# sangminwoo/Temporal-Span-Proposal-Network-VidVRD

Measured on AMD Instinct MI355X. Metric: tracklet-pairs/sec scored (N=32, T=150, D=2048), higher is better.
Workload: dtype f32

## Files before the change

temporal-span-proposal-network-vidvrd_amd/csrc/tspn_device.h:

```cpp
#pragma once
#include <hip/hip_runtime.h>

namespace tspn_dev {

typedef float f32x2 __attribute__((ext_vector_type(2)));
typedef float f32x4 __attribute__((ext_vector_type(4)));
typedef float f32x16 __attribute__((ext_vector_type(16)));
typedef __bf16 bf16x2 __attribute__((ext_vector_type(2)));
typedef __bf16 bf16x4 __attribute__((ext_vector_type(4)));
typedef __bf16 bf16x8 __attribute__((ext_vector_type(8)));
typedef _Float16 f16x8 __attribute__((ext_vector_type(8)));
typedef short s16x2 __attribute__((ext_vector_type(2)));
typedef unsigned u32x4 __attribute__((ext_vector_type(4)));

template <int AUX = 0>
__device__ __forceinline__ void glds16(const void* g, void* l) {
  __builtin_amdgcn_global_load_lds((const __attribute__((address_space(1))) void*)g,
                                   (__attribute__((address_space(3))) void*)l, 16, 0, AUX);
}
__device__ __forceinline__ void glds4(const void* g, void* l) {
  __builtin_amdgcn_global_load_lds((const __attribute__((address_space(1))) void*)g,
                                   (__attribute__((address_space(3))) void*)l, 4, 0, 0);
}

constexpr int kBufferFlags = 0x00020000;
constexpr int kBufferUnbounded = 0x7fffffff;
__device__ __forceinline__ __amdgpu_buffer_rsrc_t buffer_rsrc(const void* p, int bytes) {
  return __builtin_amdgcn_make_buffer_rsrc(const_cast<void*>(p), 0, bytes, kBufferFlags);
}
__device__ __forceinline__ __amdgpu_buffer_rsrc_t buffer_rsrc_unbounded(const void* p) {
  return buffer_rsrc(p, kBufferUnbounded);
}

__device__ __forceinline__ void bglds16(__amdgpu_buffer_rsrc_t rsrc, unsigned voff, int soff, void* l) {
  __builtin_amdgcn_raw_ptr_buffer_load_lds(rsrc, (__attribute__((address_space(3))) void*)l, 16, (int)voff, soff, 0, 0);
}

template <int OFF>
__device__ __forceinline__ void load_wfrag(f32x4& dst, unsigned lane_off, const char* base) {
  asm volatile("global_load_dwordx4 %0, %1, %2 offset:%3" : "=v"(dst) : "v"(lane_off), "s"(base), "n"(OFF) : "memory");
}
template <int VM>
__device__ __forceinline__ void wait_w(f32x4& r) {
  asm volatile("s_waitcnt vmcnt(%1)" : "+v"(r) : "n"(VM));
}
template <int VM>
__device__ __forceinline__ void wait_w(f32x4& r0, f32x4& r1) {
  asm volatile("s_waitcnt vmcnt(%2)" : "+v"(r0), "+v"(r1) : "n"(VM));
}
template <int N>
__device__ __forceinline__ void wait_vmcnt() {
  asm volatile("s_waitcnt vmcnt(%0)" ::"n"(N) : "memory");
}

__device__ __forceinline__ int xcd_remap(int id, int n) {
  const int q8 = n >> 3, r8 = n & 7, xcd = id & 7;
  return (xcd < r8 ? xcd * (q8 + 1) : r8 * (q8 + 1) + (xcd - r8) * q8) + (id >> 3);
}
__device__ __forceinline__ void grouped_tile(int wg, int GM, int tiles_m, int tiles_n, int& tile_m, int& tile_n) {
  const int group_sz = GM * tiles_n;
  const int group = wg / group_sz;
  const int first_m = group * GM;
  const int gm = min(GM, tiles_m - first_m);
  const int in_group = wg - group * group_sz;
  tile_m = first_m + in_group % gm;
  tile_n = in_group / gm;
}

}
```

temporal-span-proposal-network-vidvrd_amd/csrc/tspn_wino63.hip:

```cpp
#include <algorithm>
#include <atomic>
#include <type_traits>

#include "tspn_common.h"
#include "tspn_device.h"

namespace {

using namespace tspn_dev;

constexpr int NW = 4;
constexpr int THREADS = 64 * NW;
constexpr int BM = 128;
constexpr int ST = 32;
constexpr int SWG = 64;
constexpr int KC = 8;
constexpr int NJ = 8;
constexpr int VROW = ST * 4;
constexpr int VCH = 2 * NJ * VROW;
constexpr int VHALF = 4 * VCH;
constexpr int VSS = 2 * VHALF;
constexpr int NVB = 2;
constexpr int NPIECE = 16;
constexpr size_t SMEM_BYTES = sizeof(float) * NVB * VSS;
// ... 177 lines not shown
    if (JP == 1) { load_wfrag<2048>(ap[2], aoff, base); load_wfrag<3072>(ap[3], aoff, base); }
    if (JP == 2) { load_wfrag<0>(ap[4], aoff, base + 4096); load_wfrag<1024>(ap[5], aoff, base + 4096); }
    if (JP == 3) { load_wfrag<2048>(ap[6], aoff, base + 4096); load_wfrag<3072>(ap[7], aoff, base + 4096); }
  };
  using P0 = std::integral_constant<int, 0>;
  using P1 = std::integral_constant<int, 1>;
  using P2 = std::integral_constant<int, 2>;
  using P3 = std::integral_constant<int, 3>;
  auto mfma_pair = [&](const f32x4* ap, int ja, int jb, int S1, int slot) {
#pragma unroll
    for (int e = 0; e < 4; ++e) {
      acc[0][ja] = __builtin_amdgcn_mfma_f32_32x32x2f32(ap[ja][e], v[0][ja][e], acc[0][ja], 0, 0, 0);
      acc[0][jb] = __builtin_amdgcn_mfma_f32_32x32x2f32(ap[jb][e], v[0][jb][e], acc[0][jb], 0, 0, 0);
      acc[1][ja] = __builtin_amdgcn_mfma_f32_32x32x2f32(ap[ja][e], v[1][ja][e], acc[1][ja], 0, 0, 0);
      if (S1 >= 0) {
        __builtin_amdgcn_sched_barrier(0);
        stage_piece(S1, 4 * slot + e);
        __builtin_amdgcn_sched_barrier(0);
      }
      acc[1][jb] = __builtin_amdgcn_mfma_f32_32x32x2f32(ap[jb][e], v[1][jb][e], acc[1][jb], 0, 0, 0);
    }
  };

#pragma unroll
  for (int k = 0; k < NPIECE; ++k) stage_piece(0, k);
  asm volatile("s_waitcnt vmcnt(0)" ::: "memory");
  __syncthreads();
#pragma unroll
  for (int j = 0; j < NJ; ++j) load_v(vlane, 0, j);
  load_a_pair(a[0], P0{}, abase); load_a_pair(a[0], P1{}, abase); load_a_pair(a[0], P2{}, abase); load_a_pair(a[0], P3{}, abase);
  abase += NJ * 1024;
  load_a_pair(a[1], P0{}, abase); load_a_pair(a[1], P1{}, abase); load_a_pair(a[1], P2{}, abase); load_a_pair(a[1], P3{}, abase);
  abase += NJ * 1024;
  __builtin_amdgcn_sched_barrier(0);

  auto chunk_body = [&](auto cl_tag, const float* vcur, const float* vnext, int S, auto has1_tag, auto has2_tag,
                        auto more_tag) {
    constexpr int CL = decltype(cl_tag)::value;
    constexpr bool HAS1 = decltype(has1_tag)::value;
    constexpr bool HAS2 = decltype(has2_tag)::value;
    constexpr bool MORE = decltype(more_tag)::value;
    constexpr int PAR = CL & 1;
    constexpr int N1 = (HAS1 ? 8 : 0) + ((MORE && CL == 1) ? NPIECE : 0);
    constexpr int N2 = (MORE && CL == 2) ? 6 : 2;
    constexpr int N0 = (HAS2 ? 2 : 0) + ((MORE && CL == 0) ? 4 : 0);
    const int S1 = (MORE && CL == 0) ? S + 1 : -1;
    const float* vn = CL == 3 ? vnext : vcur;
    constexpr int NCL = (CL + 1) & 3;
    f32x4* ap = a[PAR];
    wait_w<3 * N2 + N1>(ap[0], ap[1]);
    mfma_pair(ap, 0, 1, S1, 0);
    if (HAS2) load_a_pair(ap, P0{}, abase);
    if (HAS1) { load_v(vn, NCL, 0); load_v(vn, NCL, 1); }
    __builtin_amdgcn_sched_barrier(0);
    wait_w<2 * N2 + N1 + N0>(ap[2], ap[3]);
    mfma_pair(ap, 2, 3, S1, 1);
    if (HAS2) load_a_pair(ap, P1{}, abase);
    if (HAS1) { load_v(vn, NCL, 2); load_v(vn, NCL, 3); }
    __builtin_amdgcn_sched_barrier(0);
    wait_w<N2 + N1 + 2 * N0>(ap[4], ap[5]);
    mfma_pair(ap, 4, 5, S1, 2);
    if (HAS2) load_a_pair(ap, P2{}, abase);
    if (HAS1) { load_v(vn, NCL, 4); load_v(vn, NCL, 5); }
    __builtin_amdgcn_sched_barrier(0);
    wait_w<N1 + 3 * N0>(ap[6], ap[7]);
    mfma_pair(ap, 6, 7, S1, 3);
    if (HAS2) {
      load_a_pair(ap, P3{}, abase);
      abase += NJ * 1024;
    }
    if (HAS1) { load_v(vn, NCL, 6); load_v(vn, NCL, 7); }
    __builtin_amdgcn_sched_barrier(0);
    if (MORE && CL == 2) {
      asm volatile("s_waitcnt lgkmcnt(0)" ::: "memory");
      __builtin_amdgcn_s_barrier();
      __builtin_amdgcn_sched_barrier(0);
    }
  };
  {
    using TT = std::true_type;
    using FF = std::false_type;
    using C0 = std::integral_constant<int, 0>;
    using C1 = std::integral_constant<int, 1>;
    using C2 = std::integral_constant<int, 2>;
    using C3 = std::integral_constant<int, 3>;
    int S = 0;
    for (; S + 1 < nsuper; ++S) {
      const float* vcur = vlane + (S & 1) * VSS;
      const float* vnext = vlane + ((S + 1) & 1) * VSS;
      chunk_body(C0{}, vcur, vnext, S, TT{}, TT{}, TT{});
      chunk_body(C1{}, vcur, vnext, S, TT{}, TT{}, TT{});
      chunk_body(C2{}, vcur, vnext, S, TT{}, TT{}, TT{});
      chunk_body(C3{}, vcur, vnext, S, TT{}, TT{}, TT{});
    }
    const float* vcur = vlane + (S & 1) * VSS;
    chunk_body(C0{}, vcur, vcur, S, TT{}, TT{}, FF{});
    chunk_body(C1{}, vcur, vcur, S, TT{}, TT{}, FF{});
    chunk_body(C2{}, vcur, vcur, S, TT{}, FF{}, FF{});
    chunk_body(C3{}, vcur, vcur, S, FF{}, FF{}, FF{});
  }

#pragma unroll
  for (int cb = 0; cb < 2; ++cb) {
    const int64_t Sx = S0 + ST * cb + li;
    if (Sx < nsext) {
      const int64_t b = Sx / nq;
      const int q = (int)(Sx - b * nq);
      const int t = 6 * q;
      float* ycol = y + (b * M) * (int64_t)ldy + t;
#pragma unroll
      for (int e = 0; e < 16; ++e) {
        const int m = m0 + wave * 32 + (e & 3) + 8 * (e >> 2) + 4 * kh;
        if (m < M) {
          const float p12 = acc[cb][1][e] + acc[cb][2][e], m12 = acc[cb][1][e] - acc[cb][2][e];
          const float p34 = acc[cb][3][e] + acc[cb][4][e], m34 = acc[cb][3][e] - acc[cb][4][e];
          const float p56 = acc[cb][5][e] + acc[cb][6][e], m56 = acc[cb][5][e] - acc[cb][6][e];
          float o[6];
          o[0] = acc[cb][0][e] + p12 + p34 + p56;
          o[1] = m12 + 2.f * m34 + 0.5f * m56;
          o[2] = p12 + 4.f * p34 + 0.25f * p56;
          o[3] = m12 + 8.f * m34 + 0.125f * m56;
          o[4] = p12 + 16.f * p34 + 0.0625f * p56;
          o[5] = m12 + 32.f * m34 + 0.03125f * m56 + acc[cb][7][e];
          if (bias != nullptr) {
            const float bb = bias[m];
#pragma unroll
            for (int i = 0; i < 6; ++i) o[i] += bb;
          }
          if (relu) {
#pragma unroll
            for (int i = 0; i < 6; ++i) o[i] = tspn::relu_f32(o[i]);
          }
          float* dst = ycol + (int64_t)m * ldy;
          if (vec2) {
            *reinterpret_cast<f32x2*>(dst) = f32x2{o[0], o[1]};
            *reinterpret_cast<f32x2*>(dst + 2) = f32x2{o[2], o[3]};
            *reinterpret_cast<f32x2*>(dst + 4) = f32x2{o[4], o[5]};
          } else {
#pragma unroll
            for (int i = 0; i < 6; ++i)
              if (t + i < T) dst[i] = o[i];
          }
        }
      }
    }
  }
}

constexpr int F_BM = 256, F_BN = 256;
constexpr int F_THREADS = 512;
constexpr int F_ST = 4 * 2 * 256 * 16;
constexpr int F_NST = 4;
constexpr size_t F_SMEM = (size_t)F_NST * F_ST;
constexpr size_t F_SMEM_ALL = F_SMEM + 2 * 256 * sizeof(int);
static_assert(TSPN_WINO63_GM > 0 && TSPN_WINO63_GM < 256, "the contraction's GM argument carries the tail split and the piece form above bit 7");
constexpr size_t F_PARK_PER_TILE = (size_t)7 * F_THREADS * 128 * sizeof(float);

__device__ __forceinline__ int split_exponent(double mx) {
  if (!(mx > 0.0) || !(mx <= 1.7976931348623157e308)) return 0;
  int k;
  (void)frexp(mx, &k);
  return 15 - k;
}

__device__ __forceinline__ double wino63_u(int j, double g0, double g1, double g2) {
  switch (j) {
    case 0: return g0;
    case 1: return -2.0 / 9.0 * (g0 + g1 + g2);
    case 2: return -2.0 / 9.0 * (g0 - g1 + g2);
    case 3: return g0 / 90.0 + g1 / 45.0 + 2.0 * g2 / 45.0;
    case 4: return g0 / 90.0 - g1 / 45.0 + 2.0 * g2 / 45.0;
    case 5: return (32.0 * g0 + 16.0 * g1 + 8.0 * g2) / 45.0;
    case 6: return (32.0 * g0 - 16.0 * g1 + 8.0 * g2) / 45.0;
    default: return g2;
  }
}

__global__ void pack_wino63_frag_kernel(const float* __restrict__ W, int64_t M, int64_t Cin, int64_t split,
                                        int16_t* __restrict__ out) {
  const int64_t Mp = split ? 2 * M : M, Cp = split ? split : Cin;
  const int64_t ncg = Cp / 8;
  const int64_t o = blockIdx.x * (int64_t)blockDim.x + threadIdx.x;
  if (o >= NJ * Mp) return;
  const int j = (int)(o / Mp);
  const int64_t m = o - j * Mp;
  const float* g = (split && m >= M) ? W + ((m - M) * Cin + split) * 3 : W + (m * Cin) * 3;
  double mx = 0.0;
  for (int64_t c = 0; c < Cp; ++c) {
    const double u = fabs(wino63_u(j, g[3 * c], g[3 * c + 1], g[3 * c + 2]));
    mx = (u > mx || u != u) ? u : mx;
  }
  const int e = split_exponent(mx);
  int16_t* pj = out + (int64_t)j * (2 * ncg + 1) * Mp * 8;
  for (int64_t cg = 0; cg < ncg; ++cg) {
    f16x8 hi, lo;
#pragma unroll
    for (int i = 0; i < 8; ++i) {
      const int64_t c = 8 * cg + i;
      const double u = ldexp(wino63_u(j, g[3 * c], g[3 * c + 1], g[3 * c + 2]), e);
      const _Float16 h = (_Float16)(float)u;
      hi[i] = h;
      lo[i] = (_Float16)(float)(u - (double)(float)h);
    }
    *reinterpret_cast<f16x8*>(pj + (cg * Mp + m) * 8) = hi;
    *reinterpret_cast<f16x8*>(pj + ((ncg + cg) * Mp + m) * 8) = lo;
  }
  *reinterpret_cast<int4*>(pj + (2 * ncg * Mp + m) * 8) = int4{e, 0, 0, 0};
}

__global__ __launch_bounds__(256) void wino63_input_transform_kernel(
    const float* __restrict__ x, _Float16* __restrict__ Vh, int* __restrict__ Ve, int T, int Cin, int nq,
    int64_t nsext, int64_t nsp2, int64_t ncols, unsigned long long* __restrict__ hot) {
  __shared__ float red[4][8][NJ];
  const int tid = threadIdx.x, lane = tid & 63, wave = tid >> 6;
  const int s = tid & 7, cgs = tid >> 3;
  const int64_t S = (int64_t)blockIdx.x * 8 + s;
  const bool ok = S < nsext;
  const int64_t b = ok ? S / nq : 0;
  const int q = ok ? (int)(S - b * nq) : 0;
  const int ncg = Cin >> 3;
  auto transform = [&](int cg, f32x4 (&V)[2][8], bool want_max, float& xmax) {
#pragma unroll
    for (int h = 0; h < 2; ++h) {
      f32x4 d[8];
      wino63_load_sextet(x, b, q, T, Cin, ncols, ok, 8 * cg + 4 * h, d);
      if (want_max) wino63_absmax_own_frames(d, xmax);
      wino63_bt(d, V[h]);
    }
  };
  float cmax[NJ];
#pragma unroll
  for (int j = 0; j < NJ; ++j) cmax[j] = 0.f;
  float xm = 0.f;
  for (int cg = cgs; cg < ncg; cg += 32) {
    f32x4 V[2][8];
    transform(cg, V, hot != nullptr, xm);
#pragma unroll
    for (int j = 0; j < NJ; ++j)
#pragma unroll
      for (int h = 0; h < 2; ++h)
        cmax[j] = __builtin_elementwise_maximum(
            __builtin_elementwise_maximum(cmax[j], __builtin_elementwise_maximum(fabsf(V[h][j][0]), fabsf(V[h][j][1]))),
            __builtin_elementwise_maximum(fabsf(V[h][j][2]), fabsf(V[h][j][3])));
  }
  if (hot)
    wino63_hot_publish(hot, ((unsigned long long)__float_as_uint(xm) << 32) | (unsigned)(ok ? S : 0),
                       blockIdx.x * 4 + wave);
#pragma unroll
  for (int j = 0; j < NJ; ++j) {
    float m = cmax[j];
#pragma unroll
    for (int o = 8; o < 64; o <<= 1) m = __builtin_elementwise_maximum(m, __shfl_xor(m, o, 64));
    if (lane < 8) red[wave][lane][j] = m;
  }
  __syncthreads();
  int ecol[NJ];
#pragma unroll
  for (int j = 0; j < NJ; ++j) {
    const float m = __builtin_elementwise_maximum(__builtin_elementwise_maximum(red[0][s][j], red[1][s][j]),
                                                  __builtin_elementwise_maximum(red[2][s][j], red[3][s][j]));
    ecol[j] = split_exponent((double)m);
  }
  if (cgs == 0) {
#pragma unroll
    for (int j = 0; j < NJ; ++j) Ve[(int64_t)j * nsp2 + S] = ecol[j];
  }
  for (int cg = cgs; cg < ncg; cg += 32) {
    f32x4 V[2][8];
    transform(cg, V, false, xm);
#pragma unroll
    for (int j = 0; j < NJ; ++j) {
      f16x8 hi, lo;
#pragma unroll
      for (int i = 0; i < 8; ++i) {
        const float u = ldexpf(V[i >> 2][j][i & 3], ecol[j]);
        const _Float16 h = (_Float16)u;
        hi[i] = h;
        lo[i] = (_Float16)(u - (float)h);
      }
      _Float16* dst = Vh + (((int64_t)j * 2 * ncg + cg) * nsp2 + S) * 8;
      *reinterpret_cast<f16x8*>(dst) = hi;
      *reinterpret_cast<f16x8*>(dst + (int64_t)ncg * nsp2 * 8) = lo;
    }
  }
}

#ifndef TSPN_WINO63_F16X3_STAGGER
#define TSPN_WINO63_F16X3_STAGGER 1
#endif
template <int WN, bool BUF>
__device__ __forceinline__ void wino63_f16x3_tile(
    char* smem_raw, const _Float16* __restrict__ Vh, const int* __restrict__ Ve, const int16_t* __restrict__ Wp,
    const float* __restrict__ bias, float* __restrict__ y, float* __restrict__ park, int Cin, int T, int M, int nq,
    int64_t nsext, int64_t nsp2, int tile_m, int tile_n, int tiles_n, int sub, int relu, int ldy, int vec2) {
  constexpr int MI = WN;
  constexpr int BN = 64 * WN;
  constexpr int NP = 16 + 4 * WN;
  constexpr int PW = (NP + 7) / 8;
  constexpr bool EVEN = NP % 8 == 0;
  constexpr bool STAGGER = TSPN_WINO63_F16X3_STAGGER && WN == 4;
  const int m0 = tile_m * F_BM;
  const int64_t S0 = (int64_t)tile_n * F_BN + sub * BN;

  const int tid = threadIdx.x;
  const int lane = tid & 63;
  const int wave = __builtin_amdgcn_readfirstlane(tid >> 6);
  const int wm = wave / WN, wn = wave % WN;
  const int li = lane & 31, kh = lane >> 5;
  const int ncg = Cin >> 3, nk = Cin >> 4;
  const int G = NJ * nk;

  const int p0 = wave * NP / 8;
  const int npw = EVEN ? PW : (wave + 1) * NP / 8 - p0;
  const int16_t* src[PW];
  unsigned voff[PW];
  int ldst[PW];
#pragma unroll
  for (int i = 0; i < PW; ++i) {
    const int p = min(p0 + i, NP - 1);
    int64_t el;
    if (p < 16) {
      const int region = p >> 3, cgi = (p >> 2) & 1, r = 64 * (p & 3) + lane;
      el = (((int64_t)region * ncg + cgi) * M + m0 + r) * 8;
      src[i] = Wp + el;
      ldst[i] = p * 1024;
    } else {
      const int v = p - 16;
      const int region = v / (2 * WN), cgi = (v / WN) & 1, r = 64 * (v % WN) + lane;
      el = (((int64_t)region * ncg + cgi) * nsp2 + S0 + r) * 8;
      src[i] = reinterpret_cast<const int16_t*>(Vh) + el;
      ldst[i] = (2 + region) * 8192 + cgi * 4096 + (v % WN) * 1024;
    }
    voff[i] = (unsigned)(el * 2);
  }
  int ik = 0, ist = 0;
  const char* wbase = reinterpret_cast<const char*>(Wp);
  const char* vbase = reinterpret_cast<const char*>(Vh);
  auto issue = [&]() {
    char* dst = smem_raw + ist * F_ST;
#pragma unroll
    for (int i = 0; i < PW; ++i)
      if (EVEN || i < npw) {
        if (BUF) bglds16(buffer_rsrc_unbounded(p0 + i < 16 ? wbase : vbase), voff[i], 0, dst + ldst[i]);
        else glds16(src[i], dst + ldst[i]);
      }
    ist = (ist + 1) & 3;
    const bool wrap = ++ik == nk;
    if (wrap) ik = 0;
    const int64_t dw = (int64_t)M * (wrap ? 32 * nk + 48 : 32), dv = nsp2 * (wrap ? 32 * nk + 32 : 32);
    if (BUF) {
      wbase += dw;
      vbase += dv;
    } else {
#pragma unroll
      for (int i = 0; i < PW; ++i) src[i] = reinterpret_cast<const int16_t*>(reinterpret_cast<const char*>(src[i]) + (p0 + i < 16 ? dw : dv));
    }
  };
  auto wait_stages = [&](auto ahead_tag) {
    constexpr int AHEAD = decltype(ahead_tag)::value;
    if (EVEN || npw == PW) wait_vmcnt<AHEAD * PW>(); else wait_vmcnt<AHEAD * (PW - 1)>();
  };

  f32x16 acc[MI][2];
#pragma unroll
  for (int mi = 0; mi < MI; ++mi)
#pragma unroll
    for (int ni = 0; ni < 2; ++ni)
#pragma unroll
      for (int e = 0; e < 16; ++e) acc[mi][ni][e] = 0.f;

  float* my_park = park + (int64_t)(tile_m * tiles_n + tile_n) * (F_PARK_PER_TILE / sizeof(float)) +
                   (int64_t)sub * (8 * MI) * F_THREADS * 4 + tid * 4;
  int* etab = reinterpret_cast<int*>(smem_raw + F_SMEM);
  auto unscale = [&](int j) {
    if (tid < F_BM)
      etab[tid] = reinterpret_cast<const int*>(Wp + (int64_t)j * (2 * ncg + 1) * M * 8 + (int64_t)2 * ncg * M * 8)[(int64_t)(m0 + tid) * 4];
    else if (tid - F_BM < BN)
      etab[tid] = Ve[(int64_t)j * nsp2 + S0 + tid - F_BM];
    __syncthreads();
    int ec[2];
#pragma unroll
    for (int ni = 0; ni < 2; ++ni) ec[ni] = etab[F_BM + wn * 64 + ni * 32 + li];
#pragma unroll
    for (int mi = 0; mi < MI; ++mi)
#pragma unroll
      for (int e = 0; e < 16; ++e) {
        const int r = etab[wm * (32 * MI) + mi * 32 + (e & 3) + 8 * (e >> 2) + 4 * kh];
#pragma unroll
        for (int ni = 0; ni < 2; ++ni) acc[mi][ni][e] = ldexpf(acc[mi][ni][e], -(r + ec[ni]));
      }
  };

  f16x8 ah[MI], al[MI], bh[2][2], bl[2];
  const int a_off = (kh * 256 + wm * (32 * MI) + li) * 16, b_off = (kh * 256 + wn * 64 + li) * 16;
  auto read_hi = [&](int st, f16x8 (&bhn)[2]) {
    const char* s = smem_raw + st * F_ST;
#pragma unroll
    for (int mi = 0; mi < MI; ++mi) ah[mi] = *reinterpret_cast<const f16x8*>(s + a_off + mi * 512);
#pragma unroll
    for (int ni = 0; ni < 2; ++ni) bhn[ni] = *reinterpret_cast<const f16x8*>(s + 16384 + b_off + ni * 512);
  };
  auto read_lo = [&](int st) {
    const char* s = smem_raw + st * F_ST;
#pragma unroll
    for (int ni = 0; ni < 2; ++ni) bl[ni] = *reinterpret_cast<const f16x8*>(s + 24576 + b_off + ni * 512);
#pragma unroll
    for (int mi = 0; mi < MI; ++mi) al[mi] = *reinterpret_cast<const f16x8*>(s + 8192 + a_off + mi * 512);
  };
  auto group = [&](const f16x8 (&a)[MI], const f16x8 (&b)[2]) {
#pragma unroll
    for (int ni = 0; ni < 2; ++ni)
#pragma unroll
      for (int mi = 0; mi < MI; ++mi) acc[mi][ni] = __builtin_amdgcn_mfma_f32_32x32x16_f16(a[mi], b[ni], acc[mi][ni], 0, 0, 0);
  };
  auto point_end = [&](int j) {
    unscale(j);
    if (j < NJ - 1) {
#pragma unroll
      for (int mi = 0; mi < MI; ++mi)
#pragma unroll
        for (int ni = 0; ni < 2; ++ni)
#pragma unroll
          for (int eq = 0; eq < 4; ++eq) {
            const f32x4 v = {acc[mi][ni][4 * eq], acc[mi][ni][4 * eq + 1], acc[mi][ni][4 * eq + 2], acc[mi][ni][4 * eq + 3]};
            *reinterpret_cast<f32x4*>(my_park + ((int64_t)j * 32 + (mi * 2 + ni) * 4 + eq) * F_THREADS * 4) = v;
#pragma unroll
            for (int e = 0; e < 4; ++e) acc[mi][ni][4 * eq + e] = 0.f;
          }
    }
    __builtin_amdgcn_sched_barrier(0);
  };
  auto kstep = [&](int g, f16x8 (&bc)[2], f16x8 (&bn)[2], auto steady_tag) {
    constexpr bool STEADY = decltype(steady_tag)::value;
#define TSPN_MR(NM, NR)                                \
  __builtin_amdgcn_sched_group_barrier(0x008, NM, 0);  \
  __builtin_amdgcn_sched_group_barrier(0x100, NR, 0);
    group(ah, bc);
    read_lo(g & 3);
    if (WN == 4) { TSPN_MR(1, 1) TSPN_MR(1, 1) TSPN_MR(1, 1) TSPN_MR(1, 1) TSPN_MR(1, 1) TSPN_MR(1, 1) TSPN_MR(2, 0) }
    __builtin_amdgcn_sched_barrier(0);
    if (STEADY || g + 2 < G) wait_stages(std::integral_constant<int, 1>{});
    else wait_vmcnt<0>();
    __builtin_amdgcn_s_barrier();
    __builtin_amdgcn_sched_barrier(0);
    const bool more = STEADY || g + 3 < G;
    if (more && (!STAGGER || wm == 0)) issue();
    __builtin_amdgcn_sched_barrier(0);
    group(ah, bl);
    __builtin_amdgcn_sched_barrier(0);
    if (STAGGER && more && wm != 0) issue();
    __builtin_amdgcn_sched_barrier(0);
    group(al, bc);
    if (STEADY || g + 1 < G) read_hi((g + 1) & 3, bn);
    if (WN == 4 && STEADY) { TSPN_MR(2, 1) TSPN_MR(1, 1) TSPN_MR(1, 1) TSPN_MR(1, 1) TSPN_MR(1, 1) TSPN_MR(1, 1) TSPN_MR(1, 0) }
#undef TSPN_MR
    __builtin_amdgcn_sched_barrier(0);
  };

  issue();
  issue();
  issue();
  wait_stages(std::integral_constant<int, 2>{});
  __builtin_amdgcn_s_barrier();
  __builtin_amdgcn_sched_barrier(0);
  read_hi(0, bh[0]);
  int g = 0, kc = 0, jc = 0;
  auto pair = [&](auto steady_tag) {
    kstep(g, bh[0], bh[1], steady_tag);
    kstep(g + 1, bh[1], bh[0], steady_tag);
    g += 2;
    kc += 2;
    if (kc == nk) {
      point_end(jc);
      kc = 0;
      ++jc;
    }
  };
  while (g + 4 < G) pair(std::true_type{});
  while (g < G) pair(std::false_type{});

  wait_vmcnt<0>();
#pragma unroll
  for (int ni = 0; ni < 2; ++ni) {
    const int64_t Sx = S0 + wn * 64 + ni * 32 + li;
    const bool col_ok = Sx < nsext;
    const int64_t b = col_ok ? Sx / nq : 0;
    const int q = col_ok ? (int)(Sx - b * nq) : 0;
    const int t = 6 * q;
    float* ycol = y + (b * M) * (int64_t)ldy + t;
#pragma unroll
    for (int mi = 0; mi < MI; ++mi)
#pragma unroll
      for (int eq = 0; eq < 4; ++eq) {
        f32x4 P[NJ - 1];
#pragma unroll
        for (int j = 0; j < NJ - 1; ++j)
          P[j] = *reinterpret_cast<const f32x4*>(my_park + ((int64_t)j * 32 + (mi * 2 + ni) * 4 + eq) * F_THREADS * 4);
        if (!col_ok) continue;
#pragma unroll
        for (int e4 = 0; e4 < 4; ++e4) {
          const int e = 4 * eq + e4;
          const int m = m0 + wm * (32 * MI) + mi * 32 + (e & 3) + 8 * (e >> 2) + 4 * kh;
          const float p12 = P[1][e4] + P[2][e4], m12 = P[1][e4] - P[2][e4];
          const float p34 = P[3][e4] + P[4][e4], m34 = P[3][e4] - P[4][e4];
          const float p56 = P[5][e4] + P[6][e4], m56 = P[5][e4] - P[6][e4];
          float o[6];
          o[0] = P[0][e4] + p12 + p34 + p56;
          o[1] = m12 + 2.f * m34 + 0.5f * m56;
          o[2] = p12 + 4.f * p34 + 0.25f * p56;
          o[3] = m12 + 8.f * m34 + 0.125f * m56;
          o[4] = p12 + 16.f * p34 + 0.0625f * p56;
          o[5] = m12 + 32.f * m34 + 0.03125f * m56 + acc[mi][ni][e];
          if (bias != nullptr) {
            const float bb = bias[m];
#pragma unroll
            for (int i = 0; i < 6; ++i) o[i] += bb;
          }
          if (relu) {
#pragma unroll
            for (int i = 0; i < 6; ++i) o[i] = tspn::relu_f32(o[i]);
          }
          float* dst = ycol + (int64_t)m * ldy;
          if (vec2) {
            *reinterpret_cast<f32x2*>(dst) = f32x2{o[0], o[1]};
            *reinterpret_cast<f32x2*>(dst + 2) = f32x2{o[2], o[3]};
            *reinterpret_cast<f32x2*>(dst + 4) = f32x2{o[4], o[5]};
          } else {
#pragma unroll
            for (int i = 0; i < 6; ++i)
              if (t + i < T) dst[i] = o[i];
          }
        }
      }
  }
}

__global__ __launch_bounds__(F_THREADS, 1) void conv3_wino63_kernel(
    const _Float16* __restrict__ Vh, const int* __restrict__ Ve, const int16_t* __restrict__ Wp,
    const float* __restrict__ bias, float* __restrict__ y, float* __restrict__ park, int Cin, int T, int M, int nq,
    int64_t nsext, int64_t nsp2, int tiles_m, int tiles_n, int relu, int ldy, int GM, int vec2) {
  extern __shared__ __attribute__((aligned(16))) char smem_raw[];

  const int f = max((GM >> 8) & 0xff, 1);
  const bool buf = (GM >> 16) & 1;
  GM &= 0xff;
  const int tiles = tiles_m * tiles_n;
  const int nsplit = f > 1 ? ((int)gridDim.x - tiles) / (f - 1) : 0;
  const int nfull = tiles - nsplit;
  const int bid = blockIdx.x;
  int wg, sub = 0;
  if (bid < nfull) {
    wg = xcd_remap(bid, nfull);
  } else {
    const int s = xcd_remap(bid - nfull, nsplit * f);
    wg = nfull + s / f;
    sub = s - (s / f) * f;
  }
  int tile_m, tile_n;
  grouped_tile(wg, GM, tiles_m, tiles_n, tile_m, tile_n);
  auto tile = [&](auto wn_tag, auto buf_tag) {
    wino63_f16x3_tile<decltype(wn_tag)::value, decltype(buf_tag)::value>(
        smem_raw, Vh, Ve, Wp, bias, y, park, Cin, T, M, nq, nsext, nsp2, tile_m, tile_n, tiles_n, sub, relu, ldy, vec2);
  };
  auto shape = [&](auto buf_tag) {
    if (bid < nfull) tile(std::integral_constant<int, 4>{}, buf_tag);
    else if (f == 2) tile(std::integral_constant<int, 2>{}, buf_tag);
    else tile(std::integral_constant<int, 1>{}, buf_tag);
  };
  if (buf) shape(std::true_type{}); else shape(std::false_type{});
}

int64_t padded_sextets(int64_t B, int64_t T) { return tspn::ceil_div(B * tspn::ceil_div(T, 6), SWG) * SWG; }
int64_t padded_sextets_f16x3(int64_t B, int64_t T) { return tspn::ceil_div(B * tspn::ceil_div(T, 6), F_BN) * F_BN; }

struct F16x3Layout {
  size_t v, e, park, total;
};
F16x3Layout f16x3_layout(int64_t B, int64_t T, int64_t Cin, int64_t M) {
  F16x3Layout L{};
  const size_t nsp2 = (size_t)padded_sextets_f16x3(B, T);
  L.v = 0;
  L.e = tspn::align_up((size_t)NJ * 2 * Cin * nsp2 * sizeof(_Float16), 256);
  L.park = L.e + tspn::align_up((size_t)NJ * nsp2 * sizeof(int), 256);
  L.total = L.park + (size_t)tspn::ceil_div(M, F_BM) * (nsp2 / F_BN) * F_PARK_PER_TILE;
  return L;
}

int check_common(const char* what, int64_t B, int64_t T, int64_t Cin, int64_t M, int64_t ldy) {
  TSPN_REQUIRE(B >= 0 && Cin > 0 && T > 0 && M > 0 && ldy >= T && ldy < (1 << 24), TSPN_EINVAL,
               "%s: bad sizes B=%lld T=%lld Cin=%lld M=%lld ldy=%lld", what, (long long)B, (long long)T,
               (long long)Cin, (long long)M, (long long)ldy);
  TSPN_REQUIRE(tspn::wino63_supported(Cin, M), TSPN_EUNSUPPORTED,
               "%s: needs Cin %% 32 == 0, M %% 32 == 0 (Cin=%lld M=%lld)", what, (long long)Cin, (long long)M);
  TSPN_REQUIRE(Cin < (1 << 24) && T < (1 << 24) && M < (1 << 24), TSPN_EUNSUPPORTED, "%s: dimension too large", what);
  return TSPN_OK;
}

}

bool tspn::wino63_supported(int64_t Cin, int64_t M) { return Cin > 0 && M > 0 && Cin % 32 == 0 && M % 32 == 0; }

size_t tspn::wino63_workspace_bytes(int64_t B, int64_t T, int64_t Cin) {
  if (B <= 0 || T <= 0 || Cin <= 0) return 0;
  return (size_t)(Cin / 4) * NJ * (size_t)padded_sextets(B, T) * 4 * sizeof(float);
}

extern "C" size_t tspn_conv3_tc_wino63_workspace_bytes(int64_t B, int64_t T, int64_t Cin) {
  return tspn::wino63_workspace_bytes(B, T, Cin);
}

extern "C" int tspn_pack_conv3_wino63_frag_f32(const float* W, int64_t M, int64_t Cin, int64_t split, float* frag,
                                               void* stream) {
  TSPN_REQUIRE(W && frag, TSPN_EINVAL, "tspn_pack_conv3_wino63_frag_f32: null pointer");
  TSPN_REQUIRE(M > 0 && Cin > 0 && split >= 0, TSPN_EINVAL, "tspn_pack_conv3_wino63_frag_f32: bad sizes");
  TSPN_REQUIRE(split == 0 || Cin == 2 * split, TSPN_EINVAL,
               "tspn_pack_conv3_wino63_frag_f32: split=%lld requires Cin == 2*split (Cin=%lld)", (long long)split,
               (long long)Cin);
  const int64_t Mp = split ? 2 * M : M, Cp = split ? split : Cin;
  TSPN_REQUIRE(Cp % KC == 0 && Mp % 32 == 0, TSPN_EUNSUPPORTED,
               "tspn_pack_conv3_wino63_frag_f32: needs (packed) Cin %% 8 == 0 and M %% 32 == 0 (Cin=%lld M=%lld)",
               (long long)Cp, (long long)Mp);
  const int64_t total = NJ * Cp * Mp;
  const int blocks = (int)std::min<int64_t>(tspn::ceil_div(total, 256), 8192);
  hipLaunchKernelGGL(pack_wino63_frag_kernel, dim3(blocks), dim3(256), 0, TSPN_STREAM(stream), W, M, Cin, split, frag);
  return tspn::check_launch("tspn_pack_conv3_wino63_frag_f32");
}

int tspn::wino63_input_transform(const float* x, int64_t B, int64_t T, int64_t Cin, void* workspace,
                                 size_t workspace_bytes, void* stream, uint64_t* hot) {
  const char* what = "tspn_conv3_tc_wino63_f32(input transform)";
  if (int rc = check_common(what, B, T, Cin, 32, T)) return rc;
  if (B == 0) return TSPN_OK;
  TSPN_REQUIRE(x && tspn::aligned16(x), TSPN_EINVAL, "%s: x must be a 16-byte aligned pointer", what);
  const size_t need = tspn::wino63_workspace_bytes(B, T, Cin);
  TSPN_REQUIRE(workspace && workspace_bytes >= need, TSPN_EWORKSPACE, "%s: workspace %zu < %zu bytes", what,
               workspace_bytes, need);
  TSPN_REQUIRE(tspn::aligned16(workspace), TSPN_EINVAL, "%s: workspace must be 16-byte aligned",
               what);
  const int64_t nq = tspn::ceil_div(T, 6);
  const int64_t nsext = B * nq, nsp = padded_sextets(B, T);
  TSPN_REQUIRE(nsp / 32 < (1LL << 31) && Cin / 32 < 65536, TSPN_EUNSUPPORTED, "%s: grid too large", what);
  hipLaunchKernelGGL(wino63_input_transform_kernel, dim3((unsigned)(nsp / 32), (unsigned)(Cin / 32)), dim3(256), 0,
                     TSPN_STREAM(stream), x, static_cast<float*>(workspace), (int)T, (int)Cin, (int)nq, nsext, nsp,
                     B * T, reinterpret_cast<unsigned long long*>(hot));
  return tspn::check_launch(what);
}

static std::atomic<int> g_piece_form{0};

int tspn::wino63_contract(const void* workspace, int64_t B, int64_t T, int64_t Cin, const float* frag, int64_t M,
                          const float* bias, int relu, float* y, int64_t ldy, void* stream) {
  const char* what = "tspn_conv3_tc_wino63_f32";
  if (int rc = check_common(what, B, T, Cin, M, ldy)) return rc;
  if (B == 0) return TSPN_OK;
  TSPN_REQUIRE(workspace && frag && y, TSPN_EINVAL, "%s: null pointer", what);
  TSPN_REQUIRE(tspn::aligned16(frag) && (reinterpret_cast<uintptr_t>(y) & 3) == 0,
               TSPN_EUNSUPPORTED, "%s: frag must be 16-byte aligned", what);
  const int64_t nq = tspn::ceil_div(T, 6);
  const int64_t nsext = B * nq, nsp = padded_sextets(B, T);
  const int64_t tiles_m = tspn::ceil_div(M, BM), tiles_n = nsp / SWG;
  TSPN_REQUIRE(tiles_m * tiles_n < (1LL << 31), TSPN_EUNSUPPORTED, "%s: grid too large", what);
  const int vec2 = (ldy % 2 == 0) && (ldy >= 6 * nq) && ((reinterpret_cast<uintptr_t>(y) & 7) == 0);
#ifndef TSPN_WINO63_BUFV
#define TSPN_WINO63_BUFV 1
#endif
  const bool bufv = TSPN_WINO63_BUFV && tspn::wino63_workspace_bytes(B, T, Cin) < (1ull << 32) &&
                    g_piece_form.load(std::memory_order_relaxed) == 0;
  static tspn::LdsLimit lds[2];
  auto launch = [&](auto kern, tspn::LdsLimit& lim) {
    if (int rc = lim.ensure(reinterpret_cast<const void*>(kern), SMEM_BYTES, what)) return rc;
    hipLaunchKernelGGL(kern, dim3((unsigned)(tiles_m * tiles_n)), dim3(THREADS), SMEM_BYTES, TSPN_STREAM(stream),
                       static_cast<const float*>(workspace), frag, bias, y, (int)Cin, (int)T, (int)M, (int)nq, nsext, nsp,
                       (int)tiles_m, (int)tiles_n, relu, (int)ldy, TSPN_WINO63_GM, vec2);
    return tspn::check_launch(what);
  };
  return bufv ? launch(conv3_wino63_kernel<true>, lds[1]) : launch(conv3_wino63_kernel<false>, lds[0]);
}

int tspn::conv3_tc_wino63(const float* x, int64_t B, int64_t T, int64_t Cin, const float* frag, int64_t M,
                          const float* bias, int relu, float* y, int64_t ldy, void* workspace,
                          size_t workspace_bytes, void* stream) {
  if (int rc = check_common("tspn_conv3_tc_wino63_f32", B, T, Cin, M, ldy)) return rc;
  if (int rc = tspn::wino63_input_transform(x, B, T, Cin, workspace, workspace_bytes, stream)) return rc;
  return tspn::wino63_contract(workspace, B, T, Cin, frag, M, bias, relu, y, ldy, stream);
}

extern "C" int tspn_conv3_tc_wino63_set_piece_form(int form) {
  TSPN_REQUIRE(form == 0 || form == 1, TSPN_EINVAL, "tspn_conv3_tc_wino63_set_piece_form: form must be 0 or 1");
  return g_piece_form.exchange(form, std::memory_order_relaxed);
}

extern "C" int tspn_conv3_tc_wino63_f32(const float* x, int64_t B, int64_t T, int64_t Cin, const float* frag,
                                        int64_t M, const float* bias, int relu, float* y, void* workspace,
                                        size_t workspace_bytes, void* stream) {
  return tspn::conv3_tc_wino63(x, B, T, Cin, frag, M, bias, relu, y, T, workspace, workspace_bytes, stream);
}

bool tspn::wino63_f16x3_supported(int64_t Cin, int64_t M) {
  return Cin > 0 && M > 0 && Cin % 32 == 0 && M % F_BM == 0 && Cin < (1 << 24) && M < (1 << 24);
}

size_t tspn::wino63_f16x3_workspace_bytes(int64_t B, int64_t T, int64_t Cin, int64_t M) {
  if (B <= 0 || T <= 0 || Cin <= 0 || M <= 0) return 0;
  return f16x3_layout(B, T, Cin, M).total;
}

extern "C" size_t tspn_conv3_tc_wino63_f16x3_workspace_bytes(int64_t B, int64_t T, int64_t Cin, int64_t M) {
  return tspn::wino63_f16x3_workspace_bytes(B, T, Cin, M);
}

extern "C" size_t tspn_pack_conv3_wino63_f16x3_elements(int64_t M, int64_t Cin, int64_t split) {
  if (M <= 0 || Cin <= 0 || split < 0 || (split && Cin != 2 * split)) return 0;
  const int64_t Mp = split ? 2 * M : M, Cp = split ? split : Cin;
  return (size_t)NJ * (2 * (Cp / 8) + 1) * Mp * 8;
}

extern "C" int tspn_pack_conv3_wino63_f16x3(const float* W, int64_t M, int64_t Cin, int64_t split, int16_t* packed,
// ... 123 lines not shown
```

Baseline: 1.171 million.

## Defer Winograd exponent unscaling to epilogue and double-buffer park loads

Removes the per-point unscale step, which needed a __syncthreads and ldexp over the accumulators after each Winograd point. All exponents and the bias are now preloaded into LDS once by direct global-to-LDS loads, and each point's partial sums are unscaled in the epilogue. The epilogue prefetches the next fragment's parked partial sums while finishing the current one, using inline-asm stores with vmcnt accounting. Main-loop waits are raised to leave the outstanding park stores in flight. This adds LDS footprint and brittle hand-counted vmcnt logic.

```diff
diff --git a/temporal-span-proposal-network-vidvrd_amd/csrc/tspn_device.h b/temporal-span-proposal-network-vidvrd_amd/csrc/tspn_device.h
--- a/temporal-span-proposal-network-vidvrd_amd/csrc/tspn_device.h
+++ b/temporal-span-proposal-network-vidvrd_amd/csrc/tspn_device.h
@@ -12,6 +12,7 @@
 typedef _Float16 f16x8 __attribute__((ext_vector_type(8)));
 typedef short s16x2 __attribute__((ext_vector_type(2)));
 typedef unsigned u32x4 __attribute__((ext_vector_type(4)));
+typedef int i32x4 __attribute__((ext_vector_type(4)));
 
 template <int AUX = 0>
 __device__ __forceinline__ void glds16(const void* g, void* l) {
@@ -48,6 +49,16 @@
 __device__ __forceinline__ void wait_w(f32x4& r0, f32x4& r1) {
   asm volatile("s_waitcnt vmcnt(%2)" : "+v"(r0), "+v"(r1) : "n"(VM));
 }
+template <int VM>
+__device__ __forceinline__ void wait_w(f32x4 (&r)[7]) {
+  asm volatile("s_waitcnt vmcnt(%7)"
+               : "+v"(r[0]), "+v"(r[1]), "+v"(r[2]), "+v"(r[3]), "+v"(r[4]), "+v"(r[5]), "+v"(r[6])
+               : "n"(VM));
+}
+template <int OFF>
+__device__ __forceinline__ void store_f32x2(float* p, f32x2 v) {
+  asm volatile("global_store_dwordx2 %0, %1, off offset:%2" ::"v"(p), "v"(v), "n"(OFF) : "memory");
+}
 template <int N>
 __device__ __forceinline__ void wait_vmcnt() {
   asm volatile("s_waitcnt vmcnt(%0)" ::"n"(N) : "memory");
diff --git a/temporal-span-proposal-network-vidvrd_amd/csrc/tspn_wino63.hip b/temporal-span-proposal-network-vidvrd_amd/csrc/tspn_wino63.hip
--- a/temporal-span-proposal-network-vidvrd_amd/csrc/tspn_wino63.hip
+++ b/temporal-span-proposal-network-vidvrd_amd/csrc/tspn_wino63.hip
@@ -353,7 +353,9 @@
 constexpr int F_ST = 4 * 2 * 256 * 16;
 constexpr int F_NST = 4;
 constexpr size_t F_SMEM = (size_t)F_NST * F_ST;
-constexpr size_t F_SMEM_ALL = F_SMEM + 2 * 256 * sizeof(int);
+constexpr size_t F_ETAB = (size_t)NJ * 2 * 256 * sizeof(int);
+constexpr size_t F_SMEM_ALL = F_SMEM + F_ETAB + F_BM * sizeof(float);
+static_assert(F_THREADS / 64 == NJ, "wave j of the contraction fetches the exponents of point j");
 static_assert(TSPN_WINO63_GM > 0 && TSPN_WINO63_GM < 256, "the contraction's GM argument carries the tail split and the piece form above bit 7");
 constexpr size_t F_PARK_PER_TILE = (size_t)7 * F_THREADS * 128 * sizeof(float);
 
@@ -489,6 +491,9 @@
 #ifndef TSPN_WINO63_F16X3_STAGGER
 #define TSPN_WINO63_F16X3_STAGGER 1
 #endif
+#ifndef TSPN_WINO63_F16X3_EDGES
+#define TSPN_WINO63_F16X3_EDGES 3
+#endif
 template <int WN, bool BUF>
 __device__ __forceinline__ void wino63_f16x3_tile(
     char* smem_raw, const _Float16* __restrict__ Vh, const int* __restrict__ Ve, const int16_t* __restrict__ Wp,
@@ -500,6 +505,8 @@
   constexpr int PW = (NP + 7) / 8;
   constexpr bool EVEN = NP % 8 == 0;
   constexpr bool STAGGER = TSPN_WINO63_F16X3_STAGGER && WN == 4;
+  constexpr int NS = 8 * MI;
+  constexpr bool RAISED = TSPN_WINO63_F16X3_EDGES & 1, TWO_DEEP = (TSPN_WINO63_F16X3_EDGES & 2) != 0;
   const int m0 = tile_m * F_BM;
   const int64_t S0 = (int64_t)tile_n * F_BN + sub * BN;
 
@@ -537,7 +544,7 @@
   int ik = 0, ist = 0;
   const char* wbase = reinterpret_cast<const char*>(Wp);
   const char* vbase = reinterpret_cast<const char*>(Vh);
-  auto issue = [&]() {
+  auto issue = [&]() __attribute__((always_inline)) {
     char* dst = smem_raw + ist * F_ST;
 #pragma unroll
     for (int i = 0; i < PW; ++i)
@@ -557,9 +564,9 @@
       for (int i = 0; i < PW; ++i) src[i] = reinterpret_cast<const int16_t*>(reinterpret_cast<const char*>(src[i]) + (p0 + i < 16 ? dw : dv));
     }
   };
-  auto wait_stages = [&](auto ahead_tag) {
-    constexpr int AHEAD = decltype(ahead_tag)::value;
-    if (EVEN || npw == PW) wait_vmcnt<AHEAD * PW>(); else wait_vmcnt<AHEAD * (PW - 1)>();
+  auto wait_stages = [&](auto ahead_tag, auto stores_tag) __attribute__((always_inline)) {
+    constexpr int AHEAD = decltype(ahead_tag)::value, STORES = decltype(stores_tag)::value;
+    if (EVEN || npw == PW) wait_vmcnt<AHEAD * PW + STORES>(); else wait_vmcnt<AHEAD * (PW - 1) + STORES>();
   };
 
   f32x16 acc[MI][2];
@@ -573,49 +580,40 @@
   float* my_park = park + (int64_t)(tile_m * tiles_n + tile_n) * (F_PARK_PER_TILE / sizeof(float)) +
                    (int64_t)sub * (8 * MI) * F_THREADS * 4 + tid * 4;
   int* etab = reinterpret_cast<int*>(smem_raw + F_SMEM);
-  auto unscale = [&](int j) {
-    if (tid < F_BM)
-      etab[tid] = reinterpret_cast<const int*>(Wp + (int64_t)j * (2 * ncg + 1) * M * 8 + (int64_t)2 * ncg * M * 8)[(int64_t)(m0 + tid) * 4];
-    else if (tid - F_BM < BN)
-      etab[tid] = Ve[(int64_t)j * nsp2 + S0 + tid - F_BM];
-    __syncthreads();
-    int ec[2];
-#pragma unroll
-    for (int ni = 0; ni < 2; ++ni) ec[ni] = etab[F_BM + wn * 64 + ni * 32 + li];
-#pragma unroll
-    for (int mi = 0; mi < MI; ++mi)
-#pragma unroll
-      for (int e = 0; e < 16; ++e) {
-        const int r = etab[wm * (32 * MI) + mi * 32 + (e & 3) + 8 * (e >> 2) + 4 * kh];
-#pragma unroll
-        for (int ni = 0; ni < 2; ++ni) acc[mi][ni][e] = ldexpf(acc[mi][ni][e], -(r + ec[ni]));
-      }
-  };
+  float* btab = reinterpret_cast<float*>(smem_raw + F_SMEM + F_ETAB);
+  {
+    const int* er = reinterpret_cast<const int*>(Wp + ((int64_t)wave * (2 * ncg + 1) + 2 * ncg) * M * 8) + (int64_t)(m0 + lane) * 4;
+    const int* ec = Ve + (int64_t)wave * nsp2 + S0 + lane;
+#pragma unroll
+    for (int q = 0; q < 4; ++q) glds4(er + q * 256, etab + wave * 512 + q * 64);
+#pragma unroll
+    for (int q = 0; q < WN; ++q) glds4(ec + q * 64, etab + wave * 512 + F_BM + q * 64);
+    if (bias != nullptr && wave < 4) glds4(bias + m0 + wave * 64 + lane, btab + wave * 64);
+  }
 
   f16x8 ah[MI], al[MI], bh[2][2], bl[2];
   const int a_off = (kh * 256 + wm * (32 * MI) + li) * 16, b_off = (kh * 256 + wn * 64 + li) * 16;
-  auto read_hi = [&](int st, f16x8 (&bhn)[2]) {
+  auto read_hi = [&](int st, f16x8 (&bhn)[2]) __attribute__((always_inline)) {
     const char* s = smem_raw + st * F_ST;
 #pragma unroll
     for (int mi = 0; mi < MI; ++mi) ah[mi] = *reinterpret_cast<const f16x8*>(s + a_off + mi * 512);
 #pragma unroll
     for (int ni = 0; ni < 2; ++ni) bhn[ni] = *reinterpret_cast<const f16x8*>(s + 16384 + b_off + ni * 512);
   };
-  auto read_lo = [&](int st) {
+  auto read_lo = [&](int st) __attribute__((always_inline)) {
     const char* s = smem_raw + st * F_ST;
 #pragma unroll
     for (int ni = 0; ni < 2; ++ni) bl[ni] = *reinterpret_cast<const f16x8*>(s + 24576 + b_off + ni * 512);
 #pragma unroll
     for (int mi = 0; mi < MI; ++mi) al[mi] = *reinterpret_cast<const f16x8*>(s + 8192 + a_off + mi * 512);
   };
-  auto group = [&](const f16x8 (&a)[MI], const f16x8 (&b)[2]) {
+  auto group = [&](const f16x8 (&a)[MI], const f16x8 (&b)[2]) __attribute__((always_inline)) {
 #pragma unroll
     for (int ni = 0; ni < 2; ++ni)
 #pragma unroll
       for (int mi = 0; mi < MI; ++mi) acc[mi][ni] = __builtin_amdgcn_mfma_f32_32x32x16_f16(a[mi], b[ni], acc[mi][ni], 0, 0, 0);
   };
-  auto point_end = [&](int j) {
-    unscale(j);
+  auto point_end = [&](int j) __attribute__((always_inline)) {
     if (j < NJ - 1) {
 #pragma unroll
       for (int mi = 0; mi < MI; ++mi)
@@ -631,8 +629,9 @@
     }
     __builtin_amdgcn_sched_barrier(0);
   };
-  auto kstep = [&](int g, f16x8 (&bc)[2], f16x8 (&bn)[2], auto steady_tag) {
+  auto kstep = [&](int g, f16x8 (&bc)[2], f16x8 (&bn)[2], auto steady_tag, auto post_tag) __attribute__((always_inline)) {
     constexpr bool STEADY = decltype(steady_tag)::value;
+    constexpr int STORES = decltype(post_tag)::value && RAISED ? NS : 0;
 #define TSPN_MR(NM, NR)                                \
   __builtin_amdgcn_sched_group_barrier(0x008, NM, 0);  \
   __builtin_amdgcn_sched_group_barrier(0x100, NR, 0);
@@ -640,7 +639,8 @@
     read_lo(g & 3);
     if (WN == 4) { TSPN_MR(1, 1) TSPN_MR(1, 1) TSPN_MR(1, 1) TSPN_MR(1, 1) TSPN_MR(1, 1) TSPN_MR(1, 1) TSPN_MR(2, 0) }
     __builtin_amdgcn_sched_barrier(0);
-    if (STEADY || g + 2 < G) wait_stages(std::integral_constant<int, 1>{});
+    if (STEADY || g + 2 < G)
+      wait_stages(std::integral_constant<int, 1>{}, std::integral_constant<int, STORES>{});
     else wait_vmcnt<0>();
     __builtin_amdgcn_s_barrier();
     __builtin_amdgcn_sched_barrier(0);
@@ -661,78 +661,158 @@
   issue();
   issue();
   issue();
-  wait_stages(std::integral_constant<int, 2>{});
+  wait_stages(std::integral_constant<int, 2>{}, std::integral_constant<int, 0>{});
   __builtin_amdgcn_s_barrier();
   __builtin_amdgcn_sched_barrier(0);
   read_hi(0, bh[0]);
   int g = 0, kc = 0, jc = 0;
-  auto pair = [&](auto steady_tag) {
-    kstep(g, bh[0], bh[1], steady_tag);
-    kstep(g + 1, bh[1], bh[0], steady_tag);
+  auto pair = [&](auto steady_tag, auto post_tag) __attribute__((always_inline)) {
+    kstep(g, bh[0], bh[1], steady_tag, post_tag);
+    kstep(g + 1, bh[1], bh[0], steady_tag, post_tag);
     g += 2;
     kc += 2;
-    if (kc == nk) {
-      point_end(jc);
-      kc = 0;
-      ++jc;
-    }
-  };
-  while (g + 4 < G) pair(std::true_type{});
-  while (g < G) pair(std::false_type{});
+  };
+  auto end_point = [&]() __attribute__((always_inline)) {
+    point_end(jc);
+    kc = 0;
+    ++jc;
+  };
+  const std::true_type steady, post;
+  const std::false_type generic, plain;
+  while (kc < nk) pair(steady, plain);
+  end_point();
+  const int jsteady = nk > 2 ? NJ - 1 : NJ - 2;
+  while (jc < jsteady) {
+    pair(steady, post);
+    while (kc < nk) pair(steady, plain);
+    end_point();
+  }
+  while (jc < NJ) {
+    pair(generic, post);
+    while (kc < nk && g + 4 < G) pair(steady, plain);
+    while (kc < nk) pair(generic, plain);
+    end_point();
+  }
 
   wait_vmcnt<0>();
+  constexpr int NSTEP = 2 * MI * 4;
+  const char* park_base = reinterpret_cast<const char*>(my_park - tid * 4);
+  bool col_ok[2];
+  int t0[2], ec[NJ];
+  float* ycol[2];
 #pragma unroll
   for (int ni = 0; ni < 2; ++ni) {
     const int64_t Sx = S0 + wn * 64 + ni * 32 + li;
-    const bool col_ok = Sx < nsext;
-    const int64_t b = col_ok ? Sx / nq : 0;
-    const int q = col_ok ? (int)(Sx - b * nq) : 0;
-    const int t = 6 * q;
-    float* ycol = y + (b * M) * (int64_t)ldy + t;
-#pragma unroll
-    for (int mi = 0; mi < MI; ++mi)
-#pragma unroll
-      for (int eq = 0; eq < 4; ++eq) {
-        f32x4 P[NJ - 1];
-#pragma unroll
-        for (int j = 0; j < NJ - 1; ++j)
-          P[j] = *reinterpret_cast<const f32x4*>(my_park + ((int64_t)j * 32 + (mi * 2 + ni) * 4 + eq) * F_THREADS * 4);
-        if (!col_ok) continue;
-#pragma unroll
-        for (int e4 = 0; e4 < 4; ++e4) {
-          const int e = 4 * eq + e4;
-          const int m = m0 + wm * (32 * MI) + mi * 32 + (e & 3) + 8 * (e >> 2) + 4 * kh;
-          const float p12 = P[1][e4] + P[2][e4], m12 = P[1][e4] - P[2][e4];
-          const float p34 = P[3][e4] + P[4][e4], m34 = P[3][e4] - P[4][e4];
-          const float p56 = P[5][e4] + P[6][e4], m56 = P[5][e4] - P[6][e4];
-          float o[6];
-          o[0] = P[0][e4] + p12 + p34 + p56;
-          o[1] = m12 + 2.f * m34 + 0.5f * m56;
-          o[2] = p12 + 4.f * p34 + 0.25f * p56;
-          o[3] = m12 + 8.f * m34 + 0.125f * m56;
-          o[4] = p12 + 16.f * p34 + 0.0625f * p56;
-          o[5] = m12 + 32.f * m34 + 0.03125f * m56 + acc[mi][ni][e];
-          if (bias != nullptr) {
-            const float bb = bias[m];
-#pragma unroll
-            for (int i = 0; i < 6; ++i) o[i] += bb;
+    col_ok[ni] = Sx < nsext;
+    const int64_t b = col_ok[ni] ? Sx / nq : 0;
+    const int q = col_ok[ni] ? (int)(Sx - b * nq) : 0;
+    t0[ni] = 6 * q;
+    ycol[ni] = y + (b * M) * (int64_t)ldy + t0[ni];
+  }
+  auto park_off = [&](int j, int s) __attribute__((always_inline)) {
+    const int ni = s / (4 * MI), mi = (s / 4) % MI, eq = s % 4;
+    return (unsigned)((j * 32 + (mi * 2 + ni) * 4 + eq) * F_THREADS * 16 + tid * 16);
+  };
+  auto finish = [&](f32x4 (&P)[NJ - 1], int ni, int mi, int eq, auto asm_tag) __attribute__((always_inline)) {
+    constexpr bool ASM = decltype(asm_tag)::value;
+    int row = wm * (32 * MI) + mi * 32 + 8 * eq + 4 * kh;
+    asm volatile("" : "+v"(row));
+    if (mi == 0 && eq == 0) {
+#pragma unroll
+      for (int j = 0; j < NJ; ++j) ec[j] = etab[j * 512 + F_BM + wn * 64 + ni * 32 + li];
+    }
+    f32x4 u[NJ];
+#pragma unroll
+    for (int j = 0; j < NJ - 1; ++j) u[j] = P[j];
+#pragma unroll
+    for (int e4 = 0; e4 < 4; ++e4) u[NJ - 1][e4] = acc[mi][ni][4 * eq + e4];
+#pragma unroll
+    for (int j = 0; j < NJ; ++j) {
+      const i32x4 er = *reinterpret_cast<const i32x4*>(etab + j * 512 + row);
+#pragma unroll
+      for (int e4 = 0; e4 < 4; ++e4) u[j][e4] = ldexpf(u[j][e4], -(er[e4] + ec[j]));
+    }
+    f32x4 bb = {0.f, 0.f, 0.f, 0.f};
+    if (bias != nullptr) bb = *reinterpret_cast<const f32x4*>(btab + row);
+#pragma unroll
+    for (int e4 = 0; e4 < 4; ++e4) {
+      const int m = m0 + row + e4;
+      const float p12 = u[1][e4] + u[2][e4], m12 = u[1][e4] - u[2][e4];
+      const float p34 = u[3][e4] + u[4][e4], m34 = u[3][e4] - u[4][e4];
+      const float p56 = u[5][e4] + u[6][e4], m56 = u[5][e4] - u[6][e4];
+      float o[6];
+      o[0] = u[0][e4] + p12 + p34 + p56;
+      o[1] = m12 + 2.f * m34 + 0.5f * m56;
+      o[2] = p12 + 4.f * p34 + 0.25f * p56;
+      o[3] = m12 + 8.f * m34 + 0.125f * m56;
+      o[4] = p12 + 16.f * p34 + 0.0625f * p56;
+      o[5] = m12 + 32.f * m34 + 0.03125f * m56 + u[7][e4];
+      if (bias != nullptr) {
+#pragma unroll
+        for (int i = 0; i < 6; ++i) o[i] += bb[e4];
+      }
+      if (relu) {
+#pragma unroll
+        for (int i = 0; i < 6; ++i) o[i] = tspn::relu_f32(o[i]);
+      }
+      float* dst = ycol[ni] + (int64_t)m * ldy;
+      if (ASM) {
+        store_f32x2<0>(dst, f32x2{o[0], o[1]});
+        store_f32x2<8>(dst, f32x2{o[2], o[3]});
+        store_f32x2<16>(dst, f32x2{o[4], o[5]});
+      } else if (vec2) {
+        *reinterpret_cast<f32x2*>(dst) = f32x2{o[0], o[1]};
+        *reinterpret_cast<f32x2*>(dst + 2) = f32x2{o[2], o[3]};
+        *reinterpret_cast<f32x2*>(dst + 4) = f32x2{o[4], o[5]};
+      } else {
+#pragma unroll
+        for (int i = 0; i < 6; ++i)
+          if (t0[ni] + i < T) dst[i] = o[i];
+      }
+    }
+  };
+  const bool whole = __builtin_amdgcn_ballot_w64(col_ok[0] && col_ok[1]) == ~0ull;
+  if (TWO_DEEP && vec2 && whole) {
+    f32x4 P[2][NJ - 1];
+#pragma unroll
+    for (int j = 0; j < NJ - 1; ++j) load_wfrag<0>(P[0][j], park_off(j, 0), park_base);
+    auto half = [&](auto ni_tag) __attribute__((always_inline)) {
+      constexpr int ni = decltype(ni_tag)::value;
+#pragma unroll
+      for (int mi = 0; mi < MI; ++mi)
+#pragma unroll
+        for (int eq = 0; eq < 4; ++eq) {
+          const int s = (ni * MI + mi) * 4 + eq;
+          if (s + 1 < NSTEP) {
+#pragma unroll
+            for (int j = 0; j < NJ - 1; ++j) load_wfrag<0>(P[(s + 1) & 1][j], park_off(j, s + 1), park_base);
           }
-          if (relu) {
-#pragma unroll
-            for (int i = 0; i < 6; ++i) o[i] = tspn::relu_f32(o[i]);
-          }
-          float* dst = ycol + (int64_t)m * ldy;
-          if (vec2) {
-            *reinterpret_cast<f32x2*>(dst) = f32x2{o[0], o[1]};
-            *reinterpret_cast<f32x2*>(dst + 2) = f32x2{o[2], o[3]};
-            *reinterpret_cast<f32x2*>(dst + 4) = f32x2{o[4], o[5]};
-          } else {
-#pragma unroll
-            for (int i = 0; i < 6; ++i)
-              if (t + i < T) dst[i] = o[i];
-          }
+          if (s == 0) wait_w<NJ - 1>(P[0]);
+          else if (s + 1 < NSTEP) wait_w<12 + NJ - 1>(P[s & 1]);
+          else wait_w<12>(P[s & 1]);
+          finish(P[s & 1], ni, mi, eq, std::true_type{});
+          __builtin_amdgcn_sched_barrier(0);
         }
-      }
+    };
+    half(std::integral_constant<int, 0>{});
+    half(std::integral_constant<int, 1>{});
+  } else {
+    auto half = [&](auto ni_tag) __attribute__((always_inline)) {
+      constexpr int ni = decltype(ni_tag)::value;
+#pragma unroll
+      for (int mi = 0; mi < MI; ++mi)
+#pragma unroll
+        for (int eq = 0; eq < 4; ++eq) {
+          f32x4 P[NJ - 1];
+#pragma unroll
+          for (int j = 0; j < NJ - 1; ++j)
+            P[j] = *reinterpret_cast<const f32x4*>(park_base + park_off(j, (ni * MI + mi) * 4 + eq));
+          if (col_ok[ni]) finish(P, ni, mi, eq, std::false_type{});
+          __builtin_amdgcn_sched_barrier(0);
+        }
+    };
+    half(std::integral_constant<int, 0>{});
+    half(std::integral_constant<int, 1>{});
   }
 }
 
@@ -759,11 +839,11 @@
   }
   int tile_m, tile_n;
   grouped_tile(wg, GM, tiles_m, tiles_n, tile_m, tile_n);
-  auto tile = [&](auto wn_tag, auto buf_tag) {
+  auto tile = [&](auto wn_tag, auto buf_tag) __attribute__((always_inline)) {
     wino63_f16x3_tile<decltype(wn_tag)::value, decltype(buf_tag)::value>(
         smem_raw, Vh, Ve, Wp, bias, y, park, Cin, T, M, nq, nsext, nsp2, tile_m, tile_n, tiles_n, sub, relu, ldy, vec2);
   };
-  auto shape = [&](auto buf_tag) {
+  auto shape = [&](auto buf_tag) __attribute__((always_inline)) {
     if (bid < nfull) tile(std::integral_constant<int, 4>{}, buf_tag);
     else if (f == 2) tile(std::integral_constant<int, 2>{}, buf_tag);
     else tile(std::integral_constant<int, 1>{}, buf_tag);
```

Result: slower. 1.159 million (-1.1%).
